# cropinghigh/sdrpp-dvbs-demodulator

Measured on NVIDIA B200. Metric: decoded_info_gbit_s, higher is better.
Workload: dtype int8

## Files before the change

sdrpp-dvbs-demodulator_b200/csrc/api.cu:

```cuda
#include "../../include/dvbs2fec.h"

#include <algorithm>
#include <atomic>
#include <chrono>
#include <climits>
#include <condition_variable>
#include <cstdarg>
#include <cstdio>
#include <cstring>
#include <deque>
#include <map>
#include <memory>
#include <mutex>
#include <string>
#include <thread>
#include <vector>

#include <cuda_runtime.h>
#include <emmintrin.h>

#include "bch_decoder.cuh"
#include "demapper.cuh"
#include "host_tables.h"
#include "ldpc_decoder.cuh"
// ... 79 lines not shown
    DevBuf<unsigned int> arrived;
    DevBuf<uint8_t> ts;
    DevBuf<int> ts_len;
    PinBuf<unsigned int> arrived_vals;
    DevBuf<int8_t> llr;
    DevBuf<float> sym;
    DevBuf<uint8_t> idx;
    DevBuf<uint8_t> hard;
    DevBuf<int16_t> iters;
    DevBuf<int16_t> corr;
    DevBuf<uint8_t> bb;
    DevBuf<dvbs2fec_result> res;
    DevBuf<uint8_t> workspace;
    DevBuf<unsigned int> counter;
    PinBuf<uint8_t> h_in;
    PinBuf<uint8_t> h_bb;
    PinBuf<dvbs2fec_result> h_res;
    DevBuf<uint8_t> vin;
    DevBuf<uint8_t> vbb;
    DevBuf<dvbs2fec_result> vres;
    DevBuf<VcmFrame> vmeta;
    PinBuf<VcmFrame> h_vmeta;
    bool vmeta_copying = false;
    uint8_t* user_bb = nullptr;
    dvbs2fec_result* user_res = nullptr;
    int pending = 0;
    size_t bb_bytes = 0;
    bool staged_out = true;
    uint64_t tag_base = 0;
};

struct CodeDev {
    DevBuf<uint8_t> row_level;
};
struct BchTabDev {
    DevBuf<uint16_t> crc, basis;
};

struct CodeTables {
    LdpcDev ldpc{};
    BchDev bch{};
    int grid = 0;
    int hard_stride = 0;
    std::vector<uint32_t> links;
};

struct DevCtx {
    int device = 0;
    int sms = 0;
    Slot slot[2 * kSlots + 1];
    std::mutex dev_mu;
    bool dev_used = false;
    std::map<int, CodeDev> codes;
    std::map<int, BchTabDev> bch;
    DevBuf<uint16_t> gf_log[2], gf_exp[2];
    DevBuf<uint8_t> prbs;
    DevBuf<uint8_t> pl_rn;
    std::map<int, DevBuf<uint32_t>> luts;
    LdpcDev ldpc{};
    BchDev bchd{};
    DemapDev demap{};
    int grid = 0;
    std::map<int, CodeTables> vcm_codes;
    DevBuf<DemapDev> vcm_demap;
    bool vcm_demap_ok[kVcmConfigs] = {};
    ~DevCtx() {
// ... 50 lines not shown
    struct Stage {
        PinBuf<uint8_t> in, bb, ts;
        PinBuf<dvbs2fec_result> res;
        PinBuf<int> ts_len;
        int ts_taken = 0, res_taken = 0;
        bool has_ts = false;
        std::vector<uint64_t> tags;
        int n = 0, taken = 0, cap = 0;
        int kind = 0;
        int rc = 0;
        size_t kb = 0, in_bytes = 0;
        std::atomic<int> outstanding{0};
        std::chrono::steady_clock::time_point first;
    };
    struct ShareDone { dvbs2fec_handle* h; int stage; };
    Stage stages[kStages];
    ShareDone share_done[kStages];
    std::deque<int> st_free, st_ready, st_inflight, st_done;
    int st_fill = -1;
    uint64_t launch_seq = 0;
};

static int ts_args(dvbs2fec_ts_parser* p, const uint8_t* d_bb, int cnt, uint8_t* d_out, int out_cap, int* d_produced, TsArgs* out);

namespace {

int prepare_ldpc(DevCtx& d, const LdpcCode& c, const uint32_t* links, LdpcDev& L, int& grid) {
    CodeDev& cd = d.codes[c.index];
    if (!cd.row_level.p) {
        CU(cd.row_level.reserve(c.row_level.size()));
        CU(cudaMemcpy(cd.row_level.p, c.row_level.data(), c.row_level.size(), cudaMemcpyHostToDevice));
        CU(cudaStreamSynchronize(nullptr));
    }
    L.N = c.N; L.K = c.K; L.R = c.R; L.q = c.q;
    L.ngroups = c.K / kGroup;
    L.max_cnt = c.max_cnt;
    L.v2 = ldpc_use_v2(c.index);
    L.lanes2 = L.v2 && ldpc_use_lanes2(c.index) && ldpc_slot_groups_for(c.max_cnt, true) > 0;
    L.sg = ldpc_slot_groups_for(c.max_cnt, L.lanes2);
    L.chains = !L.v2 && ldpc_chains_pay_off(c.index);
    L.occ3 = ldpc_ctas_wanted3(c.index);
    if (!L.sg) return fail(DVBS2FEC_EINVAL, "no LDPC kernel for %d links per row", c.max_cnt);
    L.links = links;
    L.layer_off = c.layer_off.data();
    L.layer_nlev = c.layer_nlev.data();
    L.row_level = cd.row_level.p;
    if (int e = ldpc_prepare(L)) return fail(DVBS2FEC_ECUDA, "LDPC kernel set-up: %s", cudaGetErrorString((cudaError_t)e));
    int per_sm = ldpc_max_ctas_per_sm(L);
    if (per_sm <= 0) return fail(DVBS2FEC_ENODEV, "LDPC kernel does not fit on device %d (%s)", d.device,
                                 cudaGetErrorString(cudaGetLastError()));
    grid = d.sms * per_sm;
    return 0;
}

int prepare_bch(DevCtx& d, const LdpcCode& c, BchDev& B) {
    const int m = c.bch_m, t = c.bch_t, fi = (m == 16);
    const GfHost& gf = gf_host(m);
    if (!d.gf_log[fi].p) {
        CU(d.gf_log[fi].reserve(gf.log.size()));
        CU(d.gf_exp[fi].reserve(gf.exp.size()));
        CU(cudaMemcpy(d.gf_log[fi].p, gf.log.data(), gf.log.size() * 2, cudaMemcpyHostToDevice));
        CU(cudaStreamSynchronize(nullptr));
        CU(cudaMemcpy(d.gf_exp[fi].p, gf.exp.data(), gf.exp.size() * 2, cudaMemcpyHostToDevice));
        CU(cudaStreamSynchronize(nullptr));
    }
    BchTabDev& bt = d.bch[m * 100 + t];
    if (!bt.crc.p) {
        const BchHost& bh = bch_host(m, t);
        CU(bt.crc.reserve(bh.crc.size()));
        CU(bt.basis.reserve(bh.basis.size()));
        CU(cudaMemcpy(bt.crc.p, bh.crc.data(), bh.crc.size() * 2, cudaMemcpyHostToDevice));
        CU(cudaStreamSynchronize(nullptr));
        CU(cudaMemcpy(bt.basis.p, bh.basis.data(), bh.basis.size() * 2, cudaMemcpyHostToDevice));
        CU(cudaStreamSynchronize(nullptr));
    }
    if (!d.prbs.p) {
        const auto& seq = bb_prbs();
        CU(d.prbs.reserve(seq.size()));
        CU(cudaMemcpy(d.prbs.p, seq.data(), seq.size(), cudaMemcpyHostToDevice));
        CU(cudaStreamSynchronize(nullptr));
    }
    B.gf.m = m; B.gf.N = gf.N; B.gf.log = d.gf_log[fi].p; B.gf.exp = d.gf_exp[fi].p;
    B.t = t; B.nbch = c.K; B.kbch = c.kbch;
    B.prefix = gf.N - c.K;
// ... 812 lines not shown
    for (int k = 0; k < kStages; ++k) {
        h->share_done[k] = {h.get(), k};
        h->st_free.push_back(k);
    }
    *out = h.release();
    return 0;
}

void dvbs2fec_destroy(dvbs2fec_handle* h) {
    if (!h) return;
    {
        std::unique_lock<std::mutex> lk(h->mu);
        h->stop = true;
        h->cv_work.notify_all();
    }
    if (h->worker.joinable()) h->worker.join();
    for (auto& dp : h->devs) {
        DevCtx& d = *dp;
        cudaSetDevice(d.device);
        cudaDeviceSynchronize();
        for (int k = 0; k < 2 * kSlots + 1; ++k) {
            Slot& s = d.slot[k];
            s.llr.release(); s.sym.release(); s.idx.release(); s.hard.release(); s.iters.release(); s.corr.release();
            s.bb.release(); s.res.release(); s.workspace.release(); s.counter.release();
            s.h_in.release(); s.h_bb.release(); s.h_res.release();
            s.arrived.release(); s.arrived_vals.release();
            s.vin.release(); s.vbb.release(); s.vres.release(); s.vmeta.release(); s.h_vmeta.release();
            s.ts.release(); s.ts_len.release();
            if (s.done) cudaEventDestroy(s.done);
            if (s.armed) cudaEventDestroy(s.armed);
            if (s.copy && !(k >= 1 && k < kSlots)) cudaStreamDestroy(s.copy);
            if (s.stream) cudaStreamDestroy(s.stream);
        }
        for (auto& kv : d.codes) kv.second.row_level.release();
        for (auto& kv : d.bch) { kv.second.crc.release(); kv.second.basis.release(); }
        for (auto& kv : d.luts) kv.second.release();
        d.vcm_demap.release();
        for (int i = 0; i < 2; ++i) { d.gf_log[i].release(); d.gf_exp[i].release(); }
        d.prbs.release();
        d.pl_rn.release();
    }
    if (h->ts) dvbs2fec_ts_destroy(h->ts);
    if (h->ts_done) cudaEventDestroy(h->ts_done);
    for (auto& sp : h->spans) {
        cudaEventDestroy(sp.a);
        cudaEventDestroy(sp.b);
    }
    for (auto& S : h->stages) {
        S.in.release();
        S.bb.release();
        S.res.release();
        S.ts.release();
        S.ts_len.release();
    }
    delete h;
}

int dvbs2fec_set_modcod(dvbs2fec_handle* h, int modcod, int shortframes, int pilots, int max_trials) {
    if (!h) return fail(DVBS2FEC_EINVAL, "handle is NULL");
    ModcodCfg mc;
    if (!modcod_config(modcod, shortframes != 0, pilots != 0, &mc))
        return fail(DVBS2FEC_EINVAL, "MODCOD %d is outside 1..28", modcod);
    if (mc.code < 0)
        return fail(DVBS2FEC_EINVAL, "MODCOD %d has no %s-frame LDPC code in EN 302 307", modcod,
                    shortframes ? "short" : "normal");
    drain_queue(h);
    h->mc = mc;
// ... 777 lines not shown
```

sdrpp-dvbs-demodulator_b200/csrc/ldpc_decoder.cu:

```cuda
#include "ldpc_decoder.cuh"
#include "ldpc_variants.h"

#include <algorithm>
#include <cstdio>
#include <cstdlib>
#include <cstring>
#include <vector>

namespace s2 {

struct LdpcPlan {
    bool v2 = false;
    int threads = kLdpcThreads;
    KernelFn fn1[2] = {nullptr, nullptr};
    KernelFn2 fn2[2] = {nullptr, nullptr};
    LdpcParams p1;
    LdpcParams2 p2;
    size_t smem = 0;
};

namespace {

int env_int(const char* name, int dflt) {
    const char* e = getenv(name);
// ... 120 lines not shown
}

bool ldpc_ctas_wanted3(int code_index) {
    static const bool table[21] = {true,  true,  true,  true,  false, false, false, false, false, false, false,
                                   true,  true,  true,  true,  true,  true,  true,  true,  true,  false};
    static const int force = env_int("DVBS2FEC_LDPC_OCC3", -1);
    if (force >= 0) return force != 0;
    return code_index >= 0 && code_index < 21 && table[code_index];
}

bool ldpc_use_v2(int code_index) {
    static const bool table[21] = {true, true, true, true, true, true, true, true, true, true, true,
                                   true, true, true, true, true, true, true, true, true, true};
    static const int force = env_int("DVBS2FEC_LDPC_V2", -1);
    if (force >= 0) return force != 0;
    return code_index >= 0 && code_index < 21 && table[code_index];
}

int ldpc_slot_groups(int max_cnt) {
    const Variant* v = pick(max_cnt);
    return v ? (v->cnt + 2 + 7) / 8 : 0;
}
int ldpc_slot_groups_for(int max_cnt, bool lanes2) {
    if (!lanes2) return ldpc_slot_groups(max_cnt);
    if (!pickl(max_cnt)) return 0;
    const int dh = (max_cnt + 1) / 2 + 1;
    return 2 * ((dh + 7) / 8);
}

bool ldpc_use_lanes2(int code_index) {
    static const bool table[21] = {false, false, false, false, false, false, true,  true,  true,  true,  true,
                                   false, false, false, false, false, false, false, false, true,  true};
    static const int force = env_int("DVBS2FEC_LDPC_LANES2", -1);
    if (force >= 0) return force != 0;
    return code_index >= 0 && code_index < 21 && table[code_index];
}

int ldpc_prepare(LdpcDev& c) {
    ldpc_release(c);
    if (c.q < 1 || c.q > kMaxLayers) return (int)cudaErrorInvalidValue;
    const int nlinks = c.layer_off[c.q];
    if (nlinks > kMaxLinks) return (int)cudaErrorInvalidValue;
    LdpcPlan* pl = new LdpcPlan();
    pl->v2 = c.v2;
    cudaError_t e = cudaSuccess;
    if (c.v2) {
        pl->fn2[0] = pick_fn2(c, false);
        pl->fn2[1] = pick_fn2(c, true);
        pl->threads = c.lanes2 ? 720 : 360;
        if (!pl->fn2[0] || !pl->fn2[1] || ldpc_slot_groups_for(c.max_cnt, c.lanes2) != c.sg) {
            delete pl;
            return (int)cudaErrorInvalidValue;
        }
        LdpcParams2& p = pl->p2;
        memset(&p, 0, sizeof(p));
        p.N = c.N; p.K = c.K; p.R = c.R; p.q = c.q; p.ngroups = c.ngroups; p.sg = c.sg;
        p.ws_stride = ldpc_workspace_bytes(c);
        p.row_level = c.row_level;
        p.wait_budget = (long long)env_int("DVBS2FEC_STREAM_WAIT_S", 20) * 2000000000ll;
        for (int i = 0; i <= c.q; ++i) p.layer_off[i] = (uint16_t)c.layer_off[i];
        for (int i = 0; i < c.q; ++i) p.layer_nlev[i] = c.layer_nlev[i];
        plan_barriers(c, p.layer_sync);
        for (int i = 0; i < nlinks; ++i) {
            const uint32_t g = c.links[i] >> 16, sh = c.links[i] & 0xFFFFu;
            p.link_group[i] = (uint8_t)g;
            p.link_add[i] = (uint16_t)(720u - 2u * sh);
        }
        for (int st = 0; st < 2 && e == cudaSuccess; ++st) e = allow_max_smem(pl->fn2[st]);
    } else {
        const Variant* v = pick(c.max_cnt);
        pl->fn1[0] = pick_fn(c, false);
        pl->fn1[1] = pick_fn(c, true);
        if (!v || !pl->fn1[0] || !pl->fn1[1] || (v->cnt + 2 + 7) / 8 != c.sg) {
            delete pl;
            return (int)cudaErrorInvalidValue;
        }
        LdpcParams& p = pl->p1;
        memset(&p, 0, sizeof(p));
        p.N = c.N; p.K = c.K; p.R = c.R; p.q = c.q; p.ngroups = c.ngroups; p.sg = c.sg;
        p.ws_stride = ldpc_workspace_bytes(c);
        p.row_level = c.row_level;
        for (int i = 0; i <= c.q; ++i) p.layer_off[i] = (uint16_t)c.layer_off[i];
        for (int i = 0; i < c.q; ++i) p.layer_nlev[i] = c.layer_nlev[i];
        plan_barriers(c, p.layer_sync);
        for (int i = 0; i < nlinks; ++i) p.links[i] = c.links[i];
        plan_chains(c, p.layer_chain);
        for (int st = 0; st < 2 && e == cudaSuccess; ++st) e = allow_max_smem(pl->fn1[st]);
    }
    if (e != cudaSuccess) {
        delete pl;
        return (int)e;
    }
    pl->smem = ldpc_smem_bytes(c);
    c.plan = pl;
    return 0;
}

void ldpc_release(LdpcDev& c) {
    delete c.plan;
    c.plan = nullptr;
}
// ... 33 lines not shown
```

sdrpp-dvbs-demodulator_b200/csrc/ldpc_decoder.cuh:

```cuda
#pragma once
#include <cstdint>
#include <cuda_runtime.h>

namespace s2 {

constexpr int kLdpcThreads = 384;
constexpr int kBitWords = 13;
constexpr int16_t kLdpcItersNoInput = -2;

struct LdpcPlan;

struct LdpcDev {
    int N, K, R, q;
    int ngroups;
    int max_cnt;
    int sg;
    bool chains;
    bool occ3;
    bool v2;
    bool lanes2;
    const LdpcPlan* plan;
    const uint32_t* links;
    const int* layer_off;
    const uint8_t* layer_nlev;
    const uint8_t* row_level;
};
int ldpc_slot_groups(int max_cnt);
bool ldpc_chains_pay_off(int code_index);
bool ldpc_ctas_wanted3(int code_index);
bool ldpc_use_v2(int code_index);
bool ldpc_use_lanes2(int code_index);
int ldpc_slot_groups_for(int max_cnt, bool lanes2);
int ldpc_prepare(LdpcDev& code);
void ldpc_release(LdpcDev& code);

struct LdpcArgs {
    LdpcDev code;
    const int8_t* llr_in;
    int nframes;
    int max_trials;
    uint8_t* hard_out;
    int hard_stride;
    int16_t* iters_out;
    int8_t* llr_out;
    uint8_t* workspace;
    unsigned int* work_counter;
    const unsigned int* arrived;
};

inline size_t ldpc_workspace_bytes(const LdpcDev& c) {
    size_t b = (size_t)c.q * c.sg * 360 * 16 + (((size_t)c.R * 2 + 15) & ~(size_t)15);
    if (c.v2) b += (size_t)2 * (c.ngroups + c.q) * kBitWords * 4 + 32 + (size_t)768 * 16;
    return (b + 255) & ~(size_t)255;
}
inline size_t ldpc_smem_bytes(const LdpcDev& c) {
    if (c.v2 && c.lanes2) return (size_t)c.K * 2 + 768 + (size_t)c.q * (4 + 2 * ((2 * ((c.max_cnt + 1) / 2) + 3) & ~3)) * 4 + 64;
    if (c.v2) return (size_t)c.K * 2 + 768 + (size_t)c.q * ((1 + 2 * c.max_cnt + 3) & ~3) * 4 + 64;
    const size_t base = (size_t)c.K * 2 + (size_t)2 * (c.ngroups + c.q) * kBitWords * 4;
    return c.chains ? ((base + 15) & ~(size_t)15) + 360 * 16 + 64 : base + 64;
}

int ldpc_launch(const LdpcArgs& args, int grid, cudaStream_t stream);
int ldpc_max_ctas_per_sm(const LdpcDev& code);

}
```

sdrpp-dvbs-demodulator_b200/csrc/ldpc_v2.cuh:

```cuda
#pragma once
#include "ldpc_decoder.cuh"
#include "ldpc_variants.h"

#include <type_traits>

namespace s2 {
namespace v2 {

constexpr int kThreads = 360;

__device__ __forceinline__ uint32_t prmt(uint32_t a, uint32_t b, uint32_t sel) {
    uint32_t d;
    asm("prmt.b32 %0, %1, %2, %3;" : "=r"(d) : "r"(a), "r"(b), "r"(sel));
    return d;
}
__device__ __forceinline__ uint32_t minu2(uint32_t a, uint32_t b) {
    uint32_t d;
    asm("min.u16x2 %0, %1, %2;" : "=r"(d) : "r"(a), "r"(b));
    return d;
}
__device__ __forceinline__ uint32_t min3u2(uint32_t a, uint32_t b, uint32_t c) {
    uint32_t d;
    asm("{.reg .b32 t; min.u16x2 t, %1, %2; min.u16x2 %0, t, %3;}" : "=r"(d) : "r"(a), "r"(b), "r"(c));
    return d;
}
__device__ __forceinline__ uint32_t addmin_relu(uint32_t a, uint32_t b, uint32_t c) {
    uint32_t d;
    asm("{.reg .b32 t; add.s16x2 t, %1, %2; min.s16x2.relu %0, t, %3;}" : "=r"(d) : "r"(a), "r"(b), "r"(c));
    return d;
}
__device__ __forceinline__ uint32_t addmin(uint32_t a, uint32_t b, uint32_t c) {
    uint32_t d;
    asm("{.reg .b32 t; add.s16x2 t, %1, %2; min.s16x2 %0, t, %3;}" : "=r"(d) : "r"(a), "r"(b), "r"(c));
    return d;
}
// ... 73 lines not shown
        uint32_t t = u;
        if (!FIRST) {
            const uint32_t beta = (c & 1) ? unpack_hi(mw[c >> 1]) : unpack_lo(mw[c >> 1]);
            t = addmin_relu(u + beta, kM32, kC255);
        }
        tu[c] = t;
        a[c] = __vabsdiffu4(t, kC128);
        sx ^= t;
    }
    exclusive_min<D>(a, ex);
    const uint32_t ssx = lane_mask7(sx);
    uint32_t prev = 0;
#pragma unroll
    for (int c = 0; c < D; ++c) {
        const uint32_t om = addmin_relu(ex[c], kAllOnes, kP32);
        const uint32_t neg = lane_mask7(tu[c]) ^ ssx;
        const uint32_t bias = neg * 0xFFFEFFFFu + kP32;
        const uint32_t bm = addmin(om ^ neg, bias, kP63);
        const uint32_t un = addmin_relu(tu[c] + bm, kM32, kC255);
        uint32_t beta;
        asm("mad.lo.u32 %0, %1, %2, %3;" : "=r"(beta) : "r"(bm), "r"(m1), "r"(kP64));
        if (c < CNT) {
            if (!RAGGED || c < cnt) sts_u16(off[c], pack_pair(un));
        } else if (c == CNT) {
            pown = un;
        } else {
            psec = un;
        }
        if (c & 1)
            mw[c >> 1] = pack_two(prev, beta);
        else if (c == D - 1)
            mw[c >> 1] = prmt(beta, keep, 0x7620);
        prev = beta;
    }
}


__device__ __forceinline__ uint32_t win360(const uint32_t* H, int o) {
    int w = o >> 5, s = o & 31;
    uint32_t r = __funnelshift_r(__ldcg(H + w), __ldcg(H + w + 1), s);
    int over = o + 32 - 360;
    if (over > 0) r |= __ldcg(H) << (32 - over);
    return r;
}
__device__ __forceinline__ uint32_t harvest8(uint4 w, uint32_t& nzacc) {
    const uint32_t k80 = 0x80808080u;
    nzacc &= __vabsdiffu4(w.x, k80) + 0x7F7F7F7Fu;
    nzacc &= __vabsdiffu4(w.y, k80) + 0x7F7F7F7Fu;
    nzacc &= __vabsdiffu4(w.z, k80) + 0x7F7F7F7Fu;
    nzacc &= __vabsdiffu4(w.w, k80) + 0x7F7F7F7Fu;
    uint32_t a0 = prmt(w.x, w.y, 0x6420), b0 = prmt(w.x, w.y, 0x7531);
    uint32_t a1 = prmt(w.z, w.w, 0x6420), b1 = prmt(w.z, w.w, 0x7531);
    auto mask4 = [](uint32_t x) { return (((~x & 0x80808080u) >> 7) * 0x00204081u >> 21) & 0xFu; };
    return mask4(a0) | (mask4(a1) << 4) | (mask4(b0) << 8) | (mask4(b1) << 12);
}
template <bool GLOBAL, int THREADS>
__device__ __forceinline__ void harvest_planes(const uint4* src, int n360, uint32_t* H, int gstride, int tid,
                                               uint32_t& nzacc) {
    uint8_t* Hb = reinterpret_cast<uint8_t*>(H);
    for (int t = tid; t < n360 * 45; t += THREADS) {
        uint4 w = GLOBAL ? __ldcg(src + t) : src[t];
        uint32_t bits = harvest8(w, nzacc);
        int g = t / 45, k = t - g * 45;
        __stcg(&Hb[g * (kBitWords * 4) + k], (uint8_t)bits);
        __stcg(&Hb[(gstride + g) * (kBitWords * 4) + k], (uint8_t)(bits >> 8));
    }
// ... 136 lines not shown
    constexpr int MW = (SLOTS + 1) / 2;
    constexpr int SG = (SLOTS + 7) / 8;
    static_assert(16 * SG >= 2 * SLOTS + 2, "the message record needs two spare bytes (row level)");
    constexpr int DW = (1 + 2 * CNT + 3) & ~3;
    extern __shared__ __align__(16) uint8_t smem_raw[];
    const int q = p.q, K = p.K, N = p.N, R = p.R;
    uint16_t* vdata = reinterpret_cast<uint16_t*>(smem_raw);
    uint16_t* X = reinterpret_cast<uint16_t*>(smem_raw + (size_t)K * 2);
    uint32_t* desc = reinterpret_cast<uint32_t*>(smem_raw + (size_t)K * 2 + 768);
    __shared__ unsigned int s_pair;
    __shared__ int s_bad[2];

    const int tid = threadIdx.x;
    const int j = tid;
    const uint32_t vbase = (uint32_t)__cvta_generic_to_shared(vdata);
    uint32_t dbase = (uint32_t)__cvta_generic_to_shared(desc);
    uint32_t j2 = 2u * (uint32_t)j;
    uint32_t xaddr = (uint32_t)__cvta_generic_to_shared(X) + j2;
    uint32_t m1 = 0xFFFFFFFFu;
    uint4* wmsg = reinterpret_cast<uint4*>(p.workspace + (size_t)blockIdx.x * p.ws_stride);
    uint16_t* wpty = reinterpret_cast<uint16_t*>(p.workspace + (size_t)blockIdx.x * p.ws_stride + (size_t)q * SG * 360 * 16);
    uint32_t* HD = reinterpret_cast<uint32_t*>(reinterpret_cast<uint8_t*>(wpty) + (((size_t)R * 2 + 15) & ~(size_t)15));
    uint32_t* HP = HD + 2 * p.ngroups * kBitWords;
    {
        volatile uint4* opq = reinterpret_cast<volatile uint4*>(HP + 2 * q * kBitWords + 4) + tid;
        opq->x = j2; opq->y = xaddr; opq->z = dbase; opq->w = m1;
        j2 = opq->x; xaddr = opq->y; dbase = opq->z; m1 = opq->w;
    }
    for (int x = tid; x < q * DW; x += kThreads) {
        const int i = x / DW, w = x - i * DW;
        const int loff = p.layer_off[i], cnt = (int)p.layer_off[i + 1] - loff;
        uint32_t v = 0;
        if (w == 0) {
            v = (uint32_t)p.layer_nlev[i] | (uint32_t)p.layer_sync[i] << 8 | (uint32_t)cnt << 16;
        } else if (w <= 2 * CNT) {
            const int c = (w - 1) >> 1;
            const int k = loff + (c < cnt ? c : 0);
            v = ((w - 1) & 1) ? (uint32_t)p.link_add[k] : vbase + 720u * p.link_group[k];
        }
        desc[x] = v;
    }
    const int npairs = (p.nframes + 1) >> 1;

    for (int x = tid; x < 2 * (p.ngroups + q) * kBitWords; x += kThreads) __stcg(&HD[x], 0u);
    __shared__ unsigned int s_next;
    if (tid == 0) s_next = kNoPair;

    for (;;) {
        __syncthreads();
        if (tid == 0) {
            unsigned np = s_next;
            if (np == kNoPair) np = atomicAdd(p.work_counter, 1u);
            s_next = kNoPair;
            if (STREAMED && np < (unsigned)npairs) {
                if (!wait_arrived(p.arrived, min(2u * np + 2u, (unsigned)p.nframes), p.wait_budget)) np |= 0x80000000u;
                __threadfence();
            }
            s_pair = np;
        }
        __syncthreads();
        const unsigned pair_word = s_pair;
        const unsigned pair = pair_word & 0x7FFFFFFFu;
        if (pair >= (unsigned)npairs) break;
        const int fa = 2 * pair, fb = 2 * pair + 1;
        const bool hasB = fb < p.nframes;
        if (STREAMED && (pair_word & 0x80000000u)) {
            if (tid == 0) {
// ... 1 lines not shown
                if (hasB) p.iters_out[fb] = kLdpcItersNoInput;
            }
            continue;
        }
        const int8_t* inA = p.llr_in + (size_t)fa * N;
        const int8_t* inB = p.llr_in + (size_t)(hasB ? fb : fa) * N;

        load_pair<STREAMED, kThreads>(p, inA, inB, vdata, wpty);
        uint32_t pown = 0, psec = 0;
        {
            const uint32_t last = __ldcg(wpty + (q - 1) * 360 + j);
            X[j + 1] = (uint16_t)last;
            pown = unpack_lo(last);
            psec = unpack_lo(__ldcg(wpty + (q - 2) * 360 + j));
        }
        if (tid == 0) X[0] = 0xFFFFu;

        int live = hasB ? 3 : 1;
        uint32_t off[CNT];
        uint32_t lw0 = 0;
        auto link_addresses = [&](int i) {
            uint32_t dw[DW];
#pragma unroll
            for (int x = 0; x < DW; x += 4)
                asm volatile("ld.shared.v4.u32 {%0, %1, %2, %3}, [%4];" : "=r"(dw[x]), "=r"(dw[x + 1]), "=r"(dw[x + 2]), "=r"(dw[x + 3])
                             : "r"(dbase + (uint32_t)(i * DW + x) * 4u));
            lw0 = dw[0];
#pragma unroll
            for (int c = 0; c < CNT; ++c)
                off[c] = dw[1 + 2 * c] + addmin_u32(j2 + dw[2 + 2 * c], (uint32_t)-720);
        };
        auto screen = [&]() -> int {
            link_addresses(q - 1);
            const int cnt = (int)(lw0 >> 16);
            uint32_t sx = pown ^ psec, mn = minu2(__vabsdiffu4(pown, kC128), __vabsdiffu4(psec, kC128));
            int nl = 2;
#pragma unroll
            for (int c = 0; c < CNT; ++c) {
                if (!RAGGED || c < cnt) {
                    const uint32_t u = unpack_lo(lds_u16(off[c]));
                    sx ^= u;
                    mn = minu2(mn, __vabsdiffu4(u, kC128));
                    ++nl;
                }
            }
            if (nl & 1) sx ^= kC128;
            int bad = 0;
            if ((sx & 0x80u) || (mn & 0xFFFFu) == 0) bad |= 1;
            if ((sx & 0x800000u) || (mn >> 16) == 0) bad |= 2;
            return bad;
        };

        __syncthreads();
        int scr = screen();
        int res[2] = {-1, -1};
        for (int n = 0;; ++n) {
            int bad = (__syncthreads_or(scr & 1) ? 1 : 0) | (__syncthreads_or(scr & 2) ? 2 : 0);
            if (live & ~bad)
                bad = full_test<kThreads>(p, wpty, HP, HD, reinterpret_cast<const uint4*>(vdata), s_bad);
            int fin = 0;
            for (int f = 0; f < 2; ++f) {
                if (!(live >> f & 1)) continue;
                if (!(bad >> f & 1)) {
                    res[f] = n;
                    fin |= 1 << f;
                } else if (n == p.max_trials) {
                    fin |= 1 << f;
                }
            }
            if (fin) {
                emit_results<kThreads>(p, fin, res, fa, fb, wpty, reinterpret_cast<const uint4*>(vdata));
                if (tid == 0 && s_next == kNoPair) s_next = claim_next_pair<STREAMED>(p, (unsigned)npairs);
                live &= ~fin;
                if (live) __syncthreads();
            }
            if (!live) break;

            auto pass = [&](auto first_tag) {
                constexpr bool FIRST = decltype(first_tag)::value;
                uint32_t mw[MW];
                uint4 nxt[SG];
                uint32_t pnext = 0;
                uint32_t pprev = 0;
#pragma unroll
                for (int x = 0; x < MW; ++x) mw[x] = 0;
                uint4* rp = wmsg + j;
                uint16_t* pp = wpty + j;
                psec = unpack_lo(lds_u16(xaddr));
                pnext = __ldcg(pp);
                if (!FIRST) {
#pragma unroll
                    for (int s = 0; s < SG; ++s) nxt[s] = __ldcg(rp + s * 360);
                }
                uint32_t lev_next = (FIRST && p.layer_nlev[0] > 1) ? (uint32_t)p.row_level[j] << 24 : 0u;
                for (int i = 0; i < q; ++i) {
                    uint32_t keep = lev_next;
                    if (!FIRST) {
#pragma unroll
                        for (int s = 0; s < SG; ++s) {
                            if (4 * s + 0 < MW) mw[4 * s + 0] = nxt[s].x;
                            if (4 * s + 1 < MW) mw[4 * s + 1] = nxt[s].y;
                            if (4 * s + 2 < MW) mw[4 * s + 2] = nxt[s].z;
                            if (4 * s + 3 < MW) mw[4 * s + 3] = nxt[s].w;
                        }
                        keep = nxt[SG - 1].w;
                    }
                    pown = unpack_lo(i == q - 1 ? lds_u16(xaddr + 2) : pnext);
                    if (i + 1 < q) {
                        pnext = __ldcg(pp + 360);
                        if (!FIRST) {
#pragma unroll
                            for (int s = 0; s < SG; ++s) nxt[s] = __ldcg(rp + (SG + s) * 360);
                        }
                    }
                    link_addresses(i);
                    const int cnt = RAGGED ? (int)(lw0 >> 16) : CNT;
                    const int nlev = (int)(lw0 & 0xFFu);
                    if (FIRST) lev_next = (i + 1 < q && p.layer_nlev[i + 1] > 1) ? (uint32_t)p.row_level[(i + 1) * 360 + j] << 24 : 0u;
                    if (nlev == 1) {
                        row_update<CNT, FIRST, RAGGED>(off, cnt, mw, pown, psec, keep, m1);
                        if (lw0 & 0x100u) __syncthreads();
                    } else {
                        const int mylev = (int)(keep >> 24);
                        for (int lvl = 0; lvl < nlev; ++lvl) {
                            if (mylev == lvl) row_update<CNT, FIRST, RAGGED>(off, cnt, mw, pown, psec, keep, m1);
                            __syncthreads();
                        }
                    }
#pragma unroll
                    for (int s = 0; s < SG; ++s) {
                        uint4 o;
                        o.x = (4 * s + 0 < MW) ? mw[4 * s + 0] : 0u;
                        o.y = (4 * s + 1 < MW) ? mw[4 * s + 1] : 0u;
                        o.z = (4 * s + 2 < MW) ? mw[4 * s + 2] : 0u;
                        o.w = (4 * s + 3 < MW) ? mw[4 * s + 3] : 0u;
                        if (s == SG - 1 && 4 * s + 3 >= MW) o.w = keep & 0xFF000000u;
                        __stcg(rp + s * 360, o);
                    }
                    if (i == 0)
                        sts_u16(xaddr, pack_pair(psec));
                    else
                        __stcg(pp - 360, (uint16_t)pack_pair(psec));
                    pprev = psec;
                    psec = pown;
                    rp += SG * 360;
                    pp += 360;
                }
                psec = pprev;
                {
                    const uint16_t pk = (uint16_t)pack_pair(pown);
                    sts_u16(xaddr + 2, pk);
                    __stcg(pp - 360, pk);
// ... 20 lines not shown
```

sdrpp-dvbs-demodulator_b200/csrc/ldpc_variants.h:

```cpp
#pragma once
#include <cstdint>

namespace s2 {

constexpr int kMaxLinks = 656;
constexpr int kMaxLayers = 136;
struct LdpcParams {
    int N, K, R, q, ngroups, sg;
    int nframes, max_trials, hard_stride, pad_;
    const int8_t* llr_in;
    uint8_t* hard_out;
    int16_t* iters_out;
    int8_t* llr_out;
    uint8_t* workspace;
    unsigned long long ws_stride;
    unsigned int* work_counter;
    const unsigned int* arrived;
    const uint8_t* row_level;
    uint16_t layer_off[kMaxLayers + 1];
    uint8_t layer_nlev[kMaxLayers];
    uint8_t layer_sync[kMaxLayers];
    uint16_t layer_chain[kMaxLayers];
    uint32_t links[kMaxLinks];
};
static_assert(sizeof(LdpcParams) <= 4096, "kernel parameter block must stay within the 4 KB constant window");

using KernelFn = void (*)(const LdpcParams);
struct Variant {
    int cnt;
    KernelFn uniform[2][2][2];
    KernelFn ragged[2][2][2];
};
extern const Variant kLdpcVariantsA[], kLdpcVariantsB[], kLdpcVariantsC[], kLdpcVariantsD[];
extern const int kLdpcVariantsA_n, kLdpcVariantsB_n, kLdpcVariantsC_n, kLdpcVariantsD_n;

struct LdpcParams2 {
    int N, K, R, q, ngroups, sg;
    int nframes, max_trials, hard_stride, pad_;
    long long wait_budget;
    const int8_t* llr_in;
    uint8_t* hard_out;
    int16_t* iters_out;
    int8_t* llr_out;
    uint8_t* workspace;
    unsigned long long ws_stride;
    unsigned int* work_counter;
    const unsigned int* arrived;
    const uint8_t* row_level;
    uint16_t layer_off[kMaxLayers + 1];
    uint8_t layer_nlev[kMaxLayers];
    uint8_t layer_sync[kMaxLayers];
    uint8_t link_group[kMaxLinks];
    uint16_t link_add[kMaxLinks];
};
static_assert(sizeof(LdpcParams2) <= 4096, "kernel parameter block must stay within the 4 KB constant window");

using KernelFn2 = void (*)(const LdpcParams2);
struct Variant2 {
    int cnt;
    KernelFn2 uniform[2][2];
    KernelFn2 ragged[2][2];
};
extern const Variant2 kLdpc2VariantsA[], kLdpc2VariantsB[], kLdpc2VariantsC[], kLdpc2VariantsD[];
extern const int kLdpc2VariantsA_n, kLdpc2VariantsB_n, kLdpc2VariantsC_n, kLdpc2VariantsD_n;

struct VariantL {
    int cnt;
    KernelFn2 uniform[2];
    KernelFn2 ragged[2];
};
extern const VariantL kLdpc2lVariantsA[], kLdpc2lVariantsB[];
extern const int kLdpc2lVariantsA_n, kLdpc2lVariantsB_n;

}
```

sdrpp-dvbs-demodulator_b200/csrc/s2_codes.cpp:

```cpp
#include "s2_codes.h"

#include <algorithm>
#include <cstring>
#include <mutex>

namespace s2 {

namespace {

struct RawDesc {
    const char* tag;
    const char* name;
    int N, K, nruns;
    int deg[3], len[3];
    int off;
};

#define S2_CODE(tag, name, N, K, nruns, d0, l0, d1, l1, d2, l2, off) \
    {#tag, name, N, K, nruns, {d0, d1, d2}, {l0, l1, l2}, off},
const RawDesc kRaw[kNumCodes] = {
#include "s2_ldpc_addr.inc"
};
#undef S2_CODE
#define S2_CODE(...)
// ... 52 lines not shown
    for (int i = 0; i < c.q; ++i) {
        auto& v = per_layer[i];
        std::stable_sort(v.begin(), v.end(), [](const LayerLink& a, const LayerLink& b) { return a.group < b.group; });
        c.layer_off[i + 1] = c.layer_off[i] + (int)v.size();
        c.max_cnt = std::max(c.max_cnt, (int)v.size());
        c.links.insert(c.links.end(), v.begin(), v.end());
    }
    c.layer_nlev.assign(c.q, 1);
    c.row_level.assign((size_t)c.q * kGroup, 0);
    c.sum_levels = 0;
    std::vector<int> next_level(c.K);
    for (int i = 0; i < c.q; ++i) {
        const LayerLink* L = &c.links[c.layer_off[i]];
        int cnt = c.layer_off[i + 1] - c.layer_off[i];
        for (int k = 0; k < cnt; ++k)
            std::fill(next_level.begin() + kGroup * L[k].group, next_level.begin() + kGroup * (L[k].group + 1), 0);
        int nlev = 1;
        for (int j = 0; j < kGroup; ++j) {
            int lvl = 0;
            for (int k = 0; k < cnt; ++k) {
                int b = kGroup * L[k].group + (j - L[k].shift + kGroup) % kGroup;
                lvl = std::max(lvl, next_level[b]);
            }
            for (int k = 0; k < cnt; ++k) {
                int b = kGroup * L[k].group + (j - L[k].shift + kGroup) % kGroup;
                next_level[b] = lvl + 1;
            }
            c.row_level[(size_t)i * kGroup + j] = (uint8_t)lvl;
            nlev = std::max(nlev, lvl + 1);
        }
        c.layer_nlev[i] = (uint8_t)nlev;
        c.sum_levels += nlev;
    }
}

}

int code_index(bool shortframe, int rate) {
    if (rate < 0 || rate > 11) return -1;
    return shortframe ? kShortIdx[rate] : kNormalIdx[rate];
}

const LdpcCode& ldpc_code(int index) {
    std::call_once(g_once[index], build, index);
    return g_codes[index];
}

const RawTable& raw_table(int index) {
    std::call_once(g_raw_once, [] {
        for (int i = 0; i < kNumCodes; ++i) {
            RawTable& t = g_rawtab[i];
            t.N = kRaw[i].N;
            t.K = kRaw[i].K;
            t.nruns = kRaw[i].nruns;
            for (int k = 0; k < 3; ++k) {
                t.deg[k] = kRaw[i].deg[k];
                t.len[k] = kRaw[i].len[k];
            }
            t.addr = kS2AddrPool + kRaw[i].off;
        }
    });
    return g_rawtab[index];
}

bool modcod_config(int modcod, bool shortframes, bool pilots, ModcodCfg* out) {
    struct Row { Constellation c; Rate r; float g1, g2; };
// ... 30 lines not shown
```

sdrpp-dvbs-demodulator_b200/csrc/s2_codes.h:

```cpp
#pragma once
#include <cstdint>
#include <vector>

namespace s2 {

constexpr int kGroup = 360;
constexpr int kNumCodes = 21;

enum Rate { R1_4 = 0, R1_3, R2_5, R1_2, R3_5, R2_3, R3_4, R4_5, R5_6, R7_8, R8_9, R9_10 };
enum Constellation { QPSK = 0, PSK8 = 1, APSK16 = 2, APSK32 = 3 };

struct ModcodCfg {
    int modcod;
    bool shortframes, pilots;
    Constellation constellation;
    int bits;
    Rate rate;
    int slots;
    float g1, g2;
    int code;
};
bool modcod_config(int modcod, bool shortframes, bool pilots, ModcodCfg* out);

struct LayerLink {
    uint16_t group;
    uint16_t shift;
};

struct LdpcCode {
    const char* name;
    int index;
    bool shortframe;
    Rate rate;
    int N, K, R, q;
    int kbch, bch_t, bch_m;
    int links_total;
    int max_cnt;
    std::vector<int> layer_off;
    std::vector<LayerLink> links;
    std::vector<uint8_t> layer_nlev;
    std::vector<uint8_t> row_level;
    int sum_levels;
};

const LdpcCode& ldpc_code(int index);
int code_index(bool shortframe, int rate);

struct RawTable {
    int N, K, nruns;
    int deg[3], len[3];
    const uint16_t* addr;
};
const RawTable& raw_table(int index);

}
```

Measured before the change: 23.58.

## Spread multi-level LDPC layer rows across several lanes per row

Adds a 'wide level' path for layered LDPC check-node updates. Multi-level layers whose per-level row sets fit are processed with 2, 4 or 8 threads cooperating on each row, using shuffle reductions for min1/min2/sign. Per-level lane assignment tables are built on the host and staged through extra shared memory. The aim is to shorten the serial level chain where few rows are active per level. The cost is extra shared memory and syncs, with a runtime occupancy check that disables the path if it would lower CTAs per SM.

```diff
diff --git a/sdrpp-dvbs-demodulator_b200/csrc/api.cu b/sdrpp-dvbs-demodulator_b200/csrc/api.cu
--- a/sdrpp-dvbs-demodulator_b200/csrc/api.cu
+++ b/sdrpp-dvbs-demodulator_b200/csrc/api.cu
@@ -135,6 +135,7 @@
 
 struct CodeDev {
     DevBuf<uint8_t> row_level;
+    DevBuf<uint16_t> wide_lanes;
 };
 struct BchTabDev {
     DevBuf<uint16_t> crc, basis;
@@ -251,6 +252,11 @@
         CU(cudaMemcpy(cd.row_level.p, c.row_level.data(), c.row_level.size(), cudaMemcpyHostToDevice));
         CU(cudaStreamSynchronize(nullptr));
     }
+    if (!cd.wide_lanes.p && !c.wide_lanes.empty()) {
+        CU(cd.wide_lanes.reserve(c.wide_lanes.size()));
+        CU(cudaMemcpy(cd.wide_lanes.p, c.wide_lanes.data(), c.wide_lanes.size() * 2, cudaMemcpyHostToDevice));
+        CU(cudaStreamSynchronize(nullptr));
+    }
     L.N = c.N; L.K = c.K; L.R = c.R; L.q = c.q;
     L.ngroups = c.K / kGroup;
     L.max_cnt = c.max_cnt;
@@ -259,16 +265,24 @@
     L.sg = ldpc_slot_groups_for(c.max_cnt, L.lanes2);
     L.chains = !L.v2 && ldpc_chains_pay_off(c.index);
     L.occ3 = ldpc_ctas_wanted3(c.index);
+    L.wide = L.v2 && !L.lanes2 && ldpc_use_wide_levels(c.index) && cd.wide_lanes.p;
     if (!L.sg) return fail(DVBS2FEC_EINVAL, "no LDPC kernel for %d links per row", c.max_cnt);
     L.links = links;
     L.layer_off = c.layer_off.data();
     L.layer_nlev = c.layer_nlev.data();
     L.row_level = cd.row_level.p;
+    L.wide_level0 = c.wide_level0.data();
+    L.wide_lanes = cd.wide_lanes.p;
     if (int e = ldpc_prepare(L)) return fail(DVBS2FEC_ECUDA, "LDPC kernel set-up: %s", cudaGetErrorString((cudaError_t)e));
     int per_sm = ldpc_max_ctas_per_sm(L);
     if (per_sm <= 0) return fail(DVBS2FEC_ENODEV, "LDPC kernel does not fit on device %d (%s)", d.device,
                                  cudaGetErrorString(cudaGetLastError()));
     grid = d.sms * per_sm;
+    static const bool log = getenv("DVBS2FEC_LDPC_LOG") && atoi(getenv("DVBS2FEC_LDPC_LOG")) != 0;
+    if (log)
+        fprintf(stderr, "dvbs2fec: LDPC short %d rate %d: %s, occ3 %d, %d CTAs per SM, wide level steps %d, %d B shared\n",
+                (int)c.shortframe, (int)c.rate, !L.v2 ? "ldpc_pair_kernel" : L.lanes2 ? "ldpc_v2l_kernel" : "ldpc_v2_kernel",
+                (int)L.occ3, per_sm, (int)L.wide, (int)ldpc_smem_bytes(L));
     return 0;
 }
 
@@ -1147,7 +1161,10 @@
             if (s.copy && !(k >= 1 && k < kSlots)) cudaStreamDestroy(s.copy);
             if (s.stream) cudaStreamDestroy(s.stream);
         }
-        for (auto& kv : d.codes) kv.second.row_level.release();
+        for (auto& kv : d.codes) {
+            kv.second.row_level.release();
+            kv.second.wide_lanes.release();
+        }
         for (auto& kv : d.bch) { kv.second.crc.release(); kv.second.basis.release(); }
         for (auto& kv : d.luts) kv.second.release();
         d.vcm_demap.release();
diff --git a/sdrpp-dvbs-demodulator_b200/csrc/ldpc_decoder.cu b/sdrpp-dvbs-demodulator_b200/csrc/ldpc_decoder.cu
--- a/sdrpp-dvbs-demodulator_b200/csrc/ldpc_decoder.cu
+++ b/sdrpp-dvbs-demodulator_b200/csrc/ldpc_decoder.cu
@@ -176,6 +176,14 @@
     static const bool table[21] = {false, false, false, false, false, false, true,  true,  true,  true,  true,
                                    false, false, false, false, false, false, false, false, true,  true};
     static const int force = env_int("DVBS2FEC_LDPC_LANES2", -1);
+    if (force >= 0) return force != 0;
+    return code_index >= 0 && code_index < 21 && table[code_index];
+}
+
+bool ldpc_use_wide_levels(int code_index) {
+    static const bool table[21] = {true, true, true, true, true, true, true, true, true, true, true,
+                                   true, true, true, true, true, true, true, true, true, true};
+    static const int force = env_int("DVBS2FEC_LDPC_WIDE_LEVELS", -1);
     if (force >= 0) return force != 0;
     return code_index >= 0 && code_index < 21 && table[code_index];
 }
@@ -211,6 +219,17 @@
             p.link_add[i] = (uint16_t)(720u - 2u * sh);
         }
         for (int st = 0; st < 2 && e == cudaSuccess; ++st) e = allow_max_smem(pl->fn2[st]);
+        c.wide = c.wide && !c.lanes2;
+        if (c.wide && e == cudaSuccess) {
+            LdpcDev narrow = c;
+            narrow.wide = false;
+            int with = 0, without = 0;
+            e = cudaOccupancyMaxActiveBlocksPerMultiprocessor(&with, pl->fn2[0], pl->threads, ldpc_smem_bytes(c));
+            if (e == cudaSuccess) e = cudaOccupancyMaxActiveBlocksPerMultiprocessor(&without, pl->fn2[0], pl->threads, ldpc_smem_bytes(narrow));
+            c.wide = with >= without;
+        }
+        p.wide_lanes = c.wide ? c.wide_lanes : nullptr;
+        for (int i = 0; i < c.q; ++i) p.wide_off[i] = (c.wide && c.wide_level0[i] >= 0) ? (uint16_t)c.wide_level0[i] : kNoWide;
     } else {
         const Variant* v = pick(c.max_cnt);
         pl->fn1[0] = pick_fn(c, false);
diff --git a/sdrpp-dvbs-demodulator_b200/csrc/ldpc_decoder.cuh b/sdrpp-dvbs-demodulator_b200/csrc/ldpc_decoder.cuh
--- a/sdrpp-dvbs-demodulator_b200/csrc/ldpc_decoder.cuh
+++ b/sdrpp-dvbs-demodulator_b200/csrc/ldpc_decoder.cuh
@@ -19,17 +19,21 @@
     bool occ3;
     bool v2;
     bool lanes2;
+    bool wide;
     const LdpcPlan* plan;
     const uint32_t* links;
     const int* layer_off;
     const uint8_t* layer_nlev;
+    const int* wide_level0;
     const uint8_t* row_level;
+    const uint16_t* wide_lanes;
 };
 int ldpc_slot_groups(int max_cnt);
 bool ldpc_chains_pay_off(int code_index);
 bool ldpc_ctas_wanted3(int code_index);
 bool ldpc_use_v2(int code_index);
 bool ldpc_use_lanes2(int code_index);
+bool ldpc_use_wide_levels(int code_index);
 int ldpc_slot_groups_for(int max_cnt, bool lanes2);
 int ldpc_prepare(LdpcDev& code);
 void ldpc_release(LdpcDev& code);
@@ -55,7 +59,7 @@
 }
 inline size_t ldpc_smem_bytes(const LdpcDev& c) {
     if (c.v2 && c.lanes2) return (size_t)c.K * 2 + 768 + (size_t)c.q * (4 + 2 * ((2 * ((c.max_cnt + 1) / 2) + 3) & ~3)) * 4 + 64;
-    if (c.v2) return (size_t)c.K * 2 + 768 + (size_t)c.q * ((1 + 2 * c.max_cnt + 3) & ~3) * 4 + 64;
+    if (c.v2) return (size_t)c.K * 2 + 768 + (size_t)c.q * ((1 + 2 * c.max_cnt + 3) & ~3) * 4 + (c.wide ? (size_t)(c.max_cnt + 4) * 720 : 0) + 64;
     const size_t base = (size_t)c.K * 2 + (size_t)2 * (c.ngroups + c.q) * kBitWords * 4;
     return c.chains ? ((base + 15) & ~(size_t)15) + 360 * 16 + 64 : base + 64;
 }
diff --git a/sdrpp-dvbs-demodulator_b200/csrc/ldpc_v2.cuh b/sdrpp-dvbs-demodulator_b200/csrc/ldpc_v2.cuh
--- a/sdrpp-dvbs-demodulator_b200/csrc/ldpc_v2.cuh
+++ b/sdrpp-dvbs-demodulator_b200/csrc/ldpc_v2.cuh
@@ -1,6 +1,7 @@
 #pragma once
 #include "ldpc_decoder.cuh"
 #include "ldpc_variants.h"
+#include "s2_codes.h"
 
 #include <type_traits>
 
@@ -140,6 +141,81 @@
         else if (c == D - 1)
             mw[c >> 1] = prmt(beta, keep, 0x7620);
         prev = beta;
+    }
+}
+
+__device__ __forceinline__ uint32_t maxu2(uint32_t a, uint32_t b) {
+    uint32_t d;
+    asm("max.u16x2 %0, %1, %2;" : "=r"(d) : "r"(a), "r"(b));
+    return d;
+}
+
+constexpr int kWideRow = 0x1FF;
+template <int CNT>
+struct WideSlots {
+    static constexpr int D = CNT + 2;
+    static constexpr int T = (D + 1) / 2;
+};
+
+template <int CNT, bool FIRST, bool RAGGED>
+__device__ __forceinline__ void wide_level(uint32_t e, int j, int cnt, uint32_t dl, uint32_t ws, uint32_t m1) {
+    constexpr int D = WideSlots<CNT>::D, T = WideSlots<CNT>::T;
+    if (e & kWideWarpIdle) return;
+    const bool act = !(e & kWideIdle);
+    const int lg = (int)(e >> 12) & 3, lane = j & ((1 << lg) - 1);
+    const uint32_t r2 = 2u * (e & kWideRow);
+    uint32_t tu[T], ad[T];
+    uint32_t wb = 0;
+    uint32_t mn1 = kC255, mn2 = kC255, sx = 0;
+#pragma unroll
+    for (int t = 0; t < T; ++t) {
+        const int c = lane + (t << lg);
+        tu[t] = kC255;
+        ad[t] = 0;
+        if (act && c < D) {
+            uint32_t u = kC255;
+            if (!RAGGED || c < cnt || c >= CNT) {
+                if (c < CNT) {
+                    const uint32_t lo = lds_u32(dl + 8u * (uint32_t)c), ln = lds_u32(dl + 8u * (uint32_t)c + 4u);
+                    ad[t] = lo + addmin_u32(r2 + ln, (uint32_t)-720);
+                } else {
+                    ad[t] = ws + 720u * (uint32_t)(c + 2) + r2;
+                }
+                u = unpack_lo(lds_u16(ad[t]));
+                if (!FIRST) u = addmin_relu(u + unpack_lo(lds_u16(ws + 720u * (uint32_t)c + r2)), kM32, kC255);
+                wb |= 1u << t;
+            }
+            tu[t] = u;
+            sx ^= u;
+            const uint32_t a = __vabsdiffu4(u, kC128);
+            mn2 = minu2(mn2, maxu2(mn1, a));
+            mn1 = minu2(mn1, a);
+        }
+    }
+    const unsigned wm = (j >= 352) ? 0xFFu : 0xFFFFFFFFu;
+    for (int s = 1; s < (1 << lg); s <<= 1) {
+        const uint32_t o1 = __shfl_xor_sync(wm, mn1, s), o2 = __shfl_xor_sync(wm, mn2, s), os = __shfl_xor_sync(wm, sx, s);
+        mn2 = min3u2(maxu2(mn1, o1), mn2, o2);
+        mn1 = minu2(mn1, o1);
+        sx ^= os;
+    }
+    const uint32_t ssx = lane_mask7(sx ^ (((D - 1) & 1) ? kC128 : 0u));
+#pragma unroll
+    for (int t = 0; t < T; ++t) {
+        if (!(wb >> t & 1)) continue;
+        const int c = lane + (t << lg);
+        const uint32_t a = __vabsdiffu4(tu[t], kC128);
+        const uint32_t eq = prmt((mn1 | 0x80008000u) - a, 0, 0xBB99);
+        const uint32_t ex = mn1 ^ ((mn1 ^ mn2) & eq);
+        const uint32_t om = addmin_relu(ex, kAllOnes, kP32);
+        const uint32_t neg = lane_mask7(tu[t]) ^ ssx;
+        const uint32_t bias = neg * 0xFFFEFFFFu + kP32;
+        const uint32_t bm = addmin(om ^ neg, bias, kP63);
+        const uint32_t un = addmin_relu(tu[t] + bm, kM32, kC255);
+        uint32_t beta;
+        asm("mad.lo.u32 %0, %1, %2, %3;" : "=r"(beta) : "r"(bm), "r"(m1), "r"(kP64));
+        sts_u16(ad[t], pack_pair(un));
+        sts_u16(ws + 720u * (uint32_t)c + r2, pack_pair(beta));
     }
 }
 
@@ -342,7 +418,8 @@
         const int loff = p.layer_off[i], cnt = (int)p.layer_off[i + 1] - loff;
         uint32_t v = 0;
         if (w == 0) {
-            v = (uint32_t)p.layer_nlev[i] | (uint32_t)p.layer_sync[i] << 8 | (uint32_t)cnt << 16;
+            v = (uint32_t)p.layer_nlev[i] | (uint32_t)p.layer_sync[i] << 8 | (uint32_t)cnt << 16 |
+                (uint32_t)(p.wide_off[i] != kNoWide) << 24;
         } else if (w <= 2 * CNT) {
             const int c = (w - 1) >> 1;
             const int k = loff + (c < cnt ? c : 0);
@@ -410,7 +487,7 @@
         };
         auto screen = [&]() -> int {
             link_addresses(q - 1);
-            const int cnt = (int)(lw0 >> 16);
+            const int cnt = (int)(lw0 >> 16 & 0xFFu);
             uint32_t sx = pown ^ psec, mn = minu2(__vabsdiffu4(pown, kC128), __vabsdiffu4(psec, kC128));
             int nl = 2;
 #pragma unroll
@@ -471,6 +548,38 @@
                     for (int s = 0; s < SG; ++s) nxt[s] = __ldcg(rp + s * 360);
                 }
                 uint32_t lev_next = (FIRST && p.layer_nlev[0] > 1) ? (uint32_t)p.row_level[j] << 24 : 0u;
+                auto wide_layer = [&](int i, int nlev, int cnt, uint32_t keep) {
+                    const uint32_t ws = dbase + (uint32_t)(q * DW) * 4u;
+                    const uint32_t dl = dbase + (uint32_t)(i * DW + 1) * 4u;
+                    if (!FIRST) {
+#pragma unroll
+                        for (int c = 0; c < SLOTS; ++c) sts_u16(ws + 720u * c + j2, (c & 1) ? mw[c >> 1] >> 16 : mw[c >> 1]);
+                    }
+                    sts_u16(ws + 720u * (SLOTS + 0) + j2, pack_pair(pown));
+                    sts_u16(ws + 720u * (SLOTS + 1) + j2, pack_pair(psec));
+                    const unsigned short* wl = p.wide_lanes + (size_t)p.wide_off[i] * 360 + j;
+                    uint32_t e = __ldg(wl);
+                    uint32_t en = (nlev > 1) ? (uint32_t)__ldg(wl + 360) : (uint32_t)(kWideIdle | kWideWarpIdle);
+                    __syncthreads();
+                    for (int lvl = 0; lvl < nlev; ++lvl) {
+                        wide_level<CNT, FIRST, RAGGED>(e, j, cnt, dl, ws, m1);
+                        e = en;
+                        if (lvl + 2 < nlev) en = __ldg(wl + (lvl + 2) * 360);
+                        __syncthreads();
+                    }
+                    pown = unpack_lo(lds_u16(ws + 720u * (SLOTS + 0) + j2));
+                    psec = unpack_lo(lds_u16(ws + 720u * (SLOTS + 1) + j2));
+                    uint32_t prev = 0;
+#pragma unroll
+                    for (int c = 0; c < SLOTS; ++c) {
+                        const uint32_t v = lds_u16(ws + 720u * c + j2);
+                        if (c & 1)
+                            mw[c >> 1] = prev | v << 16;
+                        else if (c == SLOTS - 1)
+                            mw[c >> 1] = prmt(v, keep, 0x7610);
+                        prev = v;
+                    }
+                };
                 for (int i = 0; i < q; ++i) {
                     uint32_t keep = lev_next;
                     if (!FIRST) {
@@ -484,18 +593,23 @@
                         keep = nxt[SG - 1].w;
                     }
                     pown = unpack_lo(i == q - 1 ? lds_u16(xaddr + 2) : pnext);
-                    if (i + 1 < q) {
-                        pnext = __ldcg(pp + 360);
-                        if (!FIRST) {
-#pragma unroll
-                            for (int s = 0; s < SG; ++s) nxt[s] = __ldcg(rp + (SG + s) * 360);
+                    auto prefetch = [&]() {
+                        if (i + 1 < q) {
+                            pnext = __ldcg(pp + 360);
+                            if (!FIRST) {
+#pragma unroll
+                                for (int s = 0; s < SG; ++s) nxt[s] = __ldcg(rp + (SG + s) * 360);
+                            }
                         }
-                    }
+                    };
                     link_addresses(i);
-                    const int cnt = RAGGED ? (int)(lw0 >> 16) : CNT;
+                    const int cnt = RAGGED ? (int)(lw0 >> 16 & 0xFFu) : CNT;
                     const int nlev = (int)(lw0 & 0xFFu);
+                    prefetch();
                     if (FIRST) lev_next = (i + 1 < q && p.layer_nlev[i + 1] > 1) ? (uint32_t)p.row_level[(i + 1) * 360 + j] << 24 : 0u;
-                    if (nlev == 1) {
+                    if (lw0 >> 24) {
+                        wide_layer(i, nlev, cnt, keep);
+                    } else if (nlev == 1) {
                         row_update<CNT, FIRST, RAGGED>(off, cnt, mw, pown, psec, keep, m1);
                         if (lw0 & 0x100u) __syncthreads();
                     } else {
diff --git a/sdrpp-dvbs-demodulator_b200/csrc/ldpc_variants.h b/sdrpp-dvbs-demodulator_b200/csrc/ldpc_variants.h
--- a/sdrpp-dvbs-demodulator_b200/csrc/ldpc_variants.h
+++ b/sdrpp-dvbs-demodulator_b200/csrc/ldpc_variants.h
@@ -52,7 +52,10 @@
     uint8_t layer_sync[kMaxLayers];
     uint8_t link_group[kMaxLinks];
     uint16_t link_add[kMaxLinks];
+    const uint16_t* wide_lanes;
+    uint16_t wide_off[kMaxLayers];
 };
+constexpr uint16_t kNoWide = 0xFFFF;
 static_assert(sizeof(LdpcParams2) <= 4096, "kernel parameter block must stay within the 4 KB constant window");
 
 using KernelFn2 = void (*)(const LdpcParams2);
diff --git a/sdrpp-dvbs-demodulator_b200/csrc/s2_codes.cpp b/sdrpp-dvbs-demodulator_b200/csrc/s2_codes.cpp
--- a/sdrpp-dvbs-demodulator_b200/csrc/s2_codes.cpp
+++ b/sdrpp-dvbs-demodulator_b200/csrc/s2_codes.cpp
@@ -108,6 +108,29 @@
         c.layer_nlev[i] = (uint8_t)nlev;
         c.sum_levels += nlev;
     }
+    c.wide_level0.assign(c.q, -1);
+    int nwide = 0;
+    for (int i = 0; i < c.q; ++i) {
+        const int nlev = c.layer_nlev[i];
+        if (nlev < 2) continue;
+        std::vector<std::vector<int>> rows(nlev);
+        for (int j = 0; j < kGroup; ++j) rows[c.row_level[(size_t)i * kGroup + j]].push_back(j);
+        bool fits = true;
+        for (const auto& r : rows) fits = fits && 2 * (int)r.size() <= kGroup;
+        if (!fits) continue;
+        c.wide_level0[i] = nwide;
+        nwide += nlev;
+        for (const auto& r : rows) {
+            const int n = (int)r.size(), lg = 8 * n <= kGroup ? 3 : 4 * n <= kGroup ? 2 : 1;
+            const int busy_warps = (n << lg) / 32 + ((n << lg) % 32 != 0);
+            for (int t = 0; t < kGroup; ++t) {
+                uint16_t e = (uint16_t)(lg << 12);
+                if ((t >> lg) < n) e |= (uint16_t)r[t >> lg];
+                else e |= kWideIdle | (t / 32 >= busy_warps ? kWideWarpIdle : 0);
+                c.wide_lanes.push_back(e);
+            }
+        }
+    }
 }
 
 }
diff --git a/sdrpp-dvbs-demodulator_b200/csrc/s2_codes.h b/sdrpp-dvbs-demodulator_b200/csrc/s2_codes.h
--- a/sdrpp-dvbs-demodulator_b200/csrc/s2_codes.h
+++ b/sdrpp-dvbs-demodulator_b200/csrc/s2_codes.h
@@ -41,7 +41,10 @@
     std::vector<uint8_t> layer_nlev;
     std::vector<uint8_t> row_level;
     int sum_levels;
+    std::vector<int> wide_level0;
+    std::vector<uint16_t> wide_lanes;
 };
+constexpr uint16_t kWideIdle = 0x8000, kWideWarpIdle = 0x4000;
 
 const LdpcCode& ldpc_code(int index);
 int code_index(bool shortframe, int rate);
```

New measurement: 17.65, median of 6. 25.1% lower.
